# lovesh/bulletproofs-r1cs-gadgets

Measured on AMD Instinct MI355X. Metric: R1CS proofs/sec (Poseidon VSMT-4 depth-32), higher is better.
Workload: dtype int32; 1 GPU; gadget_vsmt_4 sparse-Merkle depth-32 membership (Poseidon 4:1 inverse S-box, 148 rounds); distinct_inputs_steps=9, batch_per_gpu=1024, global_batch=1024, n_multipliers=18656, padded_n=32768, constraints=43330, proof_bytes=1377, proofs_per_device_job=4096, device_jobs=3, jobs_in_flight=2, warmup_steps_run=5, ipa_unfold_rounds=4, table_window_bits=11, table_windows=23, table_format=1, table_bytes=197767468800

## Files before the change

bulletproofs-r1cs-gadgets_amd/csrc/ipa.hpp:

```cpp
#pragma once
#include "msm_run.hpp"
static void* host_stage_alloc(size_t n);
static void host_stage_free(void* p);

struct IpaIO {
    const bpr1cs_gens* g;
    uint32_t B, N, lgN, unfold;
    strobe* tr;
    sc* a;
    sc* bb;
    sc* cG;
    sc* cH;
    const sc* qw;
    const ge* qpt;
    uint8_t* LR;
    sc* uk;
    const uint8_t* hs_tab = nullptr;
    const sc* hs_scal = nullptr;
    uint32_t hs_from = 0;
    dev_stream_t tail_stream{};
    uint32_t tail_rounds = 0;
    struct TailKeep {
        DevBuf<sc> a, bb, linv, cross, cpart;
        DevBuf<ge> GH, vwin, vsum, vout;
        DevBuf<ge_cached> vtab;
        DevBuf<uint32_t> vdig;
    }* tail_keep = nullptr;
    DevArena* own_arena = nullptr;
    sc* sG_pre = nullptr; sc* sH_pre = nullptr;
    IpaGeo geo;
    bool fuse_scalars = true;
    ge_cached* vtab_pre = nullptr; size_t vtab_pre_count = 0;
    dev_event_t* tail_event = nullptr;
};
struct IpaEnd {
    dev_stream_t st;
    sc* a; sc* bb;
};
static IpaEnd enqueue_ipa(const IpaIO& io, dev_stream_t st, MsmStats* stats) {
    const bpr1cs_gens* g = io.g;
    const uint32_t B = io.B, N = io.N, lgN = io.lgN;
    const uint32_t baseG = 2, baseH = 2 + g->cap;
    sc* a = io.a; sc* bb = io.bb; sc* cG = io.cG; sc* cH = io.cH;
    DevBuf<sc> cross((size_t)2 * B);
    const uint32_t r = io.unfold < lgN ? io.unfold : lgN;
    DevBuf<sc> sG, sH, cpart;
    DevBuf<ge> GH, vwin, vsum, vout, partial, partialR;
    DevBuf<ge_cached> vtab;
    DevBuf<uint32_t> vdig;
    DevBuf<sc> linv;
    MsmPlan plan;
    uint32_t M = N >> r;
    ge* GHp = nullptr; ge* vwinp = nullptr; ge* vsump = nullptr; ge* voutp = nullptr;
    ge_cached* vtabp = nullptr; uint32_t* vdigp = nullptr; sc* linvp = nullptr; sc* crossp = cross.p;
    sc* sGp = io.sG_pre; sc* sHp = io.sH_pre;
    const bool geo = io.geo.plo != nullptr;
    if ((r > 0 || (geo && lgN > 0)) && !(sGp && sHp)) { sG.alloc((size_t)N * B); sH.alloc((size_t)N * B); sGp = sG.p; sHp = sH.p; }
    const size_t s_bytes = sGp ? (size_t)N * B * sizeof(sc) : 0;
    const uint32_t facT = 1u << r;
    DevBuf<sc> fac;
    const uint32_t hfJ = N >> 8;
    DevBuf<sc> hf;
    if (geo && lgN > 0) {
        fac.alloc((size_t)6 * facT * B);
        if (hfJ) hf.alloc((size_t)2 * hfJ * B);
    }
    const bool fused = geo && B > MSM_LANE_PATH_MAX_PROOFS && io.fuse_scalars;
    MsmGeo mg;
    auto geo_scalars = [&](uint32_t k, const sc* va, const sc* vb) {
        const uint32_t lgNk = lgN - k;
        launch((uint64_t)2 * (k ? 1u << (k - 1) : 1u) * B, K_ipa_fac{fac.p, k ? io.uk + (size_t)(k - 1) * 2 * B : nullptr, io.geo.upad, B, k, facT}, st);
        const sc* hfp = nullptr;
        if (lgNk >= 8 && hfJ) {
            launch((uint64_t)2 * hfJ * B, K_ipa_hf{fac.p, io.geo.phi + (size_t)io.geo.H * B, hf.p, B, hfJ, lgNk - 8, facT}, st);
            hfp = hf.p;
        }
        if (fused) {
            mg.fac = fac.p; mg.hf = hfp; mg.lo1 = io.geo.plo + (size_t)256 * B; mg.hi1 = io.geo.phi + (size_t)io.geo.H * B;
            mg.T = facT; mg.J = hfJ; mg.Nk = N >> k; mg.lgNk = lgNk; mg.n1 = io.geo.n1;
            return;
        }
        launch((uint64_t)N * B, K_ipa_scalars_geo{va, vb, fac.p, hfp, io.geo, sGp, sHp, B, N >> k, lgNk, facT, hfJ}, st);
    };
    const uint32_t VC = 16;
    const uint32_t VC_TAIL = 4;
    bool vb_reuse = false;
    auto finisher = [&](const ge* part, uint32_t nch, const sc* c, uint8_t* out) {
        K_msm_finish f{g->tab.p, g->tc, part, c, io.qw, out, B, nch, 0};
        if (io.qpt) { f.extra2 = nullptr; f.extra_pt = io.qpt; }
        return f;
    };
    uint32_t tail_from = lgN;
    if (io.tail_rounds && io.tail_keep && io.tail_rounds < lgN) {
        tail_from = std::max(lgN - io.tail_rounds, r + 2);
        if ((tail_from - r) & 1u) tail_from++;
    }
    sc* cpartp = nullptr; size_t cpart_n = 0;
    bool handed_off = false;
    auto emit = [&](uint64_t total, const auto& f, bool wave) {
        if (wave) launch_wave(total, f, st);
        else launch(total, f, st);
    };
    for (uint32_t k = 0; k < lgN; k++) {
        uint32_t Nk = N >> k, mk = Nk >> 1;
        if (k == tail_from && k + 1 < lgN) {
            IpaIO::TailKeep& T = *io.tail_keep;
            {
                ArenaScope own(io.own_arena);
                T.a.alloc((size_t)Nk * B); T.bb.alloc((size_t)Nk * B); T.linv.alloc((size_t)2 * B); T.cross.alloc((size_t)2 * B);
                T.GH.alloc((size_t)2 * Nk * B);
                T.vtab.alloc((size_t)VB_MULT * 4 * mk * B); T.vdig.alloc((size_t)VB_WORDS * 4 * mk * B);
                T.vwin.alloc((size_t)2 * VB_WINDOWS * VC_TAIL * B); T.vsum.alloc((size_t)2 * VB_WINDOWS * B); T.vout.alloc((size_t)2 * B);
            }
            dev_d2d(T.a.p, a, (size_t)Nk * B * sizeof(sc), st);
            dev_d2d(T.bb.p, bb, (size_t)Nk * B * sizeof(sc), st);
            dev_d2d(T.linv.p, linvp, (size_t)2 * B * sizeof(sc), st);
            dev_d2d(T.GH.p, GHp, (size_t)Nk * B * sizeof(ge), st);
            dev_d2d(T.GH.p + (size_t)Nk * B, GHp + (size_t)M * B, (size_t)Nk * B * sizeof(ge), st);
            dev_zero(io.a, (size_t)N * B * sizeof(sc), st);
            dev_zero(io.bb, (size_t)N * B * sizeof(sc), st);
            if (s_bytes) { dev_zero(sGp, s_bytes, st); dev_zero(sHp, s_bytes, st); }
            if (vdig.p) dev_zero(vdig.p, vdig.bytes(), st);
            if (cpart.p) dev_zero(cpart.p, cpart.bytes(), st);
            dev_zero(cross.p, cross.bytes(), st);
            handed_off = true;
            a = T.a.p; bb = T.bb.p; linvp = T.linv.p; crossp = T.cross.p; GHp = T.GH.p; M = Nk;
            vtabp = T.vtab.p; vdigp = T.vdig.p; vwinp = T.vwin.p; vsump = T.vsum.p; voutp = T.vout.p;
            cpartp = nullptr; cpart_n = 0;
            if (io.tail_event) {
                dev_event_create(io.tail_event);
                dev_event_record(*io.tail_event, st);
                dev_stream_wait(io.tail_stream, *io.tail_event);
                st = io.tail_stream;
            }
        }
        uint32_t cchunk, CC = pick_chunks(mk, B, std::min<uint32_t>(1u << 18, sum_chunk_cap(B, 2) * B), cchunk);
        if (cpart_n < (size_t)2 * CC * B) {
            if (k >= tail_from && io.tail_keep) {
                ArenaScope own(io.own_arena);
                io.tail_keep->cpart.alloc((size_t)2 * CC * B);
                cpartp = io.tail_keep->cpart.p;
            } else {
                cpart.alloc((size_t)2 * CC * B);
                cpartp = cpart.p;
            }
            cpart_n = (size_t)2 * CC * B;
        }
        emit((uint64_t)CC * B, K_ipa_cross{a, bb, cpartp, B, mk, cchunk, CC}, false);
        launch_sum_partials((uint64_t)2 * B, K_sum_partials{cpartp, crossp, B, CC}, st);
        uint8_t* Lout = io.LR + ((size_t)k * 2 + 0) * B * 32;
        uint8_t* Rout = io.LR + ((size_t)k * 2 + 1) * B * 32;
        if (k < r) {
            if (geo) {
                geo_scalars(k, a, bb);
            } else {
                K_ipa_scalars ks{a, bb, cG, cH, sGp, sHp, B, Nk};
                if (k > 0) ks.uk_prev = io.uk + (size_t)(k - 1) * 2 * B;
                launch((uint64_t)N * B, ks, st);
            }
            uint32_t half = N / 2;
            MsmSeg gL{sGp, half, mk, Nk, mk, baseG, 0}, hL{sHp, half, mk, Nk, 0, baseH, 0};
            MsmSeg gR{sGp, half, mk, Nk, 0, baseG, 0}, hR{sHp, half, mk, Nk, mk, baseH, 0};
            if (fused) {
                gL.scal = gR.scal = a; hL.scal = hR.scal = bb;
                gL.geo = gR.geo = 1; hL.geo = hR.geo = 2;
            }
            const bool hs = k == 0 && io.hs_tab && io.hs_from < mk;
            if (hs) {
                hL.count = io.hs_from;
                gR.count = io.hs_from;
            }
            MsmPlan planR;
            MsmReq rq[2] = {{gL, hL, &partial, &plan, nullptr}, {gR, hR, &partialR, &planR, nullptr}};
            run_msm_multi(g, rq, 2, B, st, stats, fused ? &mg : nullptr);
            K_msm_finish fL = finisher(partial.p, plan.nchunks, crossp, Lout);
            if (hs) { fL.tab2 = io.hs_tab; fL.extra_b = io.hs_scal; }
            launch_finish_pair(fL, finisher(partialR.p, planR.nchunks, crossp + B, Rout), B, st);
        } else {
            if (k == r) {
                const size_t dead = r >= 1 ? (size_t)(N - M) * B * sizeof(sc) : 0;
                const size_t gh_b = (size_t)2 * M * B * sizeof(ge), vwin_b = ((size_t)2 * VB_WINDOWS * VC * B * sizeof(ge) + 255) & ~(size_t)255,
                             vdig_b = (size_t)VB_WORDS * 4 * (M / 2 ? M / 2 : 1) * B * sizeof(uint32_t);
                if (gh_b <= dead) GHp = (ge*)(io.a + (size_t)M * B);
                else { GH.alloc((size_t)2 * M * B); GHp = GH.p; }
                if (vwin_b + vdig_b <= dead) {
                    uint8_t* base = (uint8_t*)(io.bb + (size_t)M * B);
                    vwinp = (ge*)base;
                    vdigp = (uint32_t*)(base + vwin_b);
                } else {
                    vdig.alloc((size_t)VB_WORDS * 4 * (M / 2 ? M / 2 : 1) * B);
                    vwin.alloc((size_t)2 * VB_WINDOWS * VC * B);
                    vdigp = vdig.p; vwinp = vwin.p;
                }
                const sc* fG = cG; const sc* fH = cH;
                if (geo) {
                    geo_scalars(k, nullptr, nullptr);
                    fG = sGp; fH = sHp;
                }
                const uint32_t f_mont = geo ? 0u : 1u;
                if (B <= MSM_LANE_PATH_MAX_PROOFS) {
                    launch_wave((uint64_t)2 * M * B, K_ipa_fold_from_tables{g->tab.p, g->tc, fG, fH, GHp, B, M, N, baseG, baseH, geo ? 1u : 0u}, st);
                } else {
                    MsmLaunch L{};
                    L.B = B; L.nbk = (B + 63u) / 64u; L.njobs = 2;
                    const MsmSeg none{nullptr, 0, 1, 1, 0, 0, 0};
                    L.job[0] = MsmJob{{MsmSeg{fG, N, N, N, 0, baseG, f_mont}, none}, g->tab.p, g->tc, GHp, N / M, M, 1};
                    L.job[1] = MsmJob{{MsmSeg{fH, N, N, N, 0, baseH, f_mont}, none}, g->tab.p, g->tc, GHp + (size_t)M * B, N / M, M, 1};
                    if (fused) {
                        L.job[0].seg[0].scal = nullptr; L.job[0].seg[0].geo = 1;
                        L.job[1].seg[0].scal = nullptr; L.job[1].seg[0].geo = 2;
                        L.geo = mg;
                    }
                    L.wg_end[0] = M * L.nbk; L.wg_end[1] = 2 * M * L.nbk;
                    launch_msm_kernel(g, L, st, stats, (uint64_t)2 * N * B, (uint64_t)2 * N * B * g->tc.windows);
                }
                const size_t vtab_need = (size_t)VB_MULT * 4 * (M / 2 ? M / 2 : 1) * B;
                if (!(io.vtab_pre && io.vtab_pre_count >= vtab_need)) vtab.alloc(vtab_need);
                vsum.alloc((size_t)2 * VB_WINDOWS * B);
                vout.alloc((size_t)2 * B);
                linv.alloc((size_t)2 * B);
                launch((uint64_t)2 * B, K_set_one{linv.p}, st);
                vtabp = vtab.p ? vtab.p : io.vtab_pre; vsump = vsum.p; voutp = vout.p; linvp = linv.p;
            }
            const uint32_t remap = 1u;
            if (!vb_reuse) {
                const uint32_t vcmax = handed_off ? VC_TAIL : VC;
                const uint32_t vc = 2 * mk < vcmax ? 2 * mk : vcmax;
                emit((uint64_t)4 * mk * B, K_ipa_vb_tab{a, bb, GHp, linvp, vtabp, vdigp, B, mk, M}, false);
                emit((uint64_t)2 * VB_WINDOWS * vc * B, K_ipa_vb_win{vtabp, vdigp, vwinp, B, mk, vc, remap, 0}, true);
                emit((uint64_t)2 * VB_WINDOWS * B, K_ge_reduce{vwinp, vsump, B, 2 * VB_WINDOWS * vc, vc}, false);
            } else {
                const uint32_t vcmax = handed_off ? VC_TAIL : VC;
                const uint32_t m0 = 2 * mk, vc = 2 * m0 < vcmax ? 2 * m0 : vcmax;
                emit((uint64_t)4 * m0 * B, K_ipa_vb_dig2{a, bb, linvp, io.uk + (size_t)(k - 1) * 2 * B, vdigp, B, m0}, false);
                emit((uint64_t)2 * VB_WINDOWS * vc * B, K_ipa_vb_win{vtabp, vdigp, vwinp, B, m0, vc, remap, 1}, true);
                emit((uint64_t)2 * VB_WINDOWS * B, K_ge_reduce{vwinp, vsump, B, 2 * VB_WINDOWS * vc, vc}, false);
            }
            emit((uint64_t)2 * B, K_ipa_vb_horner{vsump, voutp, B, 1}, false);
            launch_finish_pair(finisher(voutp, 1, crossp, Lout), finisher(voutp + (size_t)B, 1, crossp + B, Rout), B, st);
        }
        sc* ukk = io.uk + (size_t)k * 2 * B;
        launch_transcript(B, K_transcript_LR{io.tr, Lout, ukk, B}, st);
        emit((uint64_t)mk * B, K_ipa_fold_ab{a, bb, ukk, B, mk}, false);
        if (k + 1 == r && !geo) launch((uint64_t)N * B, K_ipa_update_c{cG, cH, ukk, B, Nk}, st);
        else if (k < r) {}
        else if (!vb_reuse) {
            vb_reuse = k + 1 < lgN;
        } else {
            if (k + 1 < lgN) emit((uint64_t)2 * mk * B, K_ipa_vb_fold2{GHp, io.uk + (size_t)(k - 1) * 2 * B, ukk, linvp, vtabp, B, 2 * mk, M}, false);
            vb_reuse = false;
        }
    }
    if (!handed_off && s_bytes) {
        dev_zero(sGp, s_bytes, st);
        dev_zero(sHp, s_bytes, st);
    }
    if (handed_off) {
        IpaIO::TailKeep& T = *io.tail_keep;
        if (T.vdig.p) dev_zero(T.vdig.p, T.vdig.bytes(), st);
        if (T.cpart.p) dev_zero(T.cpart.p, T.cpart.bytes(), st);
        if (T.cross.p) dev_zero(T.cross.p, T.cross.bytes(), st);
    } else {
        if (vdig.p) dev_zero(vdig.p, vdig.bytes(), st);
        if (cpart.p) dev_zero(cpart.p, cpart.bytes(), st);
        dev_zero(cross.p, cross.bytes(), st);
    }
    return IpaEnd{st, a, bb};
}
```

bulletproofs-r1cs-gadgets_amd/csrc/kernels.hpp:

```cpp
#pragma once
#include "fe.hpp"
#include "sc.hpp"
#include "ge.hpp"
#include "merlin.hpp"
#include "msm_trace.hpp"

struct TabCfg {
    uint32_t W, windows, entries, row, per_base;
    uint32_t stride;
    HD size_t base_bytes() const { return (size_t)per_base * stride; }
};
HD inline TabCfg tab_cfg(uint32_t W) {
    TabCfg t;
    t.W = W;
    t.windows = (252 + W) / W;
    t.entries = 1u << (W - 1);
    t.row = t.entries + 1;
    t.per_base = t.windows * t.row;
    t.stride = 128;
    return t;
}
HD inline int tab_digit(const sc& s, uint32_t k, int& carry, const TabCfg& tc) {
    uint32_t bit = k * tc.W, wi = bit >> 5, sh = bit & 31;
    uint64_t two = (uint64_t)s.v[wi] | ((wi + 1 < 8) ? ((uint64_t)s.v[wi + 1] << 32) : 0);
// ... 807 lines not shown
};

struct K_ct_gather_T {
    const sc* tco;
    const sc* blind;
    sc* out;
    uint32_t B;
    HD void operator()(uint32_t g) const {
        const uint32_t k = g / B, b = g % B;
        const uint32_t ti[5] = {0, 2, 3, 4, 5};
        out[g] = tco[(size_t)ti[k] * B + b];
        out[(size_t)5 * B + g] = blind[(size_t)(3 + k) * B + b];
    }
};
struct K_ct_finish {
    const ge* partial;
    uint32_t nchunks, count;
    uint8_t* out;
    uint32_t B, m;
    HD void operator()(uint32_t g) const {
        ge acc = partial[g];
        for (uint32_t c = 1; c < nchunks; c++) acc = ge_add_ge(acc, partial[(size_t)c * count + g]);
        ge_compress(acc, out + 32 * (m ? (size_t)(g % B) * m + g / B : (size_t)g));
    }
};

struct K_transcript_T {
    strobe* tr;
    const uint8_t* Tc;
    const sc* tco;
    const sc* blind;
    const sc* wV;
    const sc* vbl_m;
    sc* chal;
    sc* txs;
    uint32_t B, m;
    uint64_t padded_n;
    const sc* t2b_pre = nullptr;
    HD void operator()(uint32_t b) const {
        strobe s = tr[b];
        merlin_append(s, "T_1", 3, Tc + ((size_t)0 * B + b) * 32, 32);
        merlin_append(s, "T_3", 3, Tc + ((size_t)1 * B + b) * 32, 32);
        merlin_append(s, "T_4", 3, Tc + ((size_t)2 * B + b) * 32, 32);
        merlin_append(s, "T_5", 3, Tc + ((size_t)3 * B + b) * 32, 32);
        merlin_append(s, "T_6", 3, Tc + ((size_t)4 * B + b) * 32, 32);
        sc u = merlin_challenge_scalar(s, "u", 1);
        sc x = merlin_challenge_scalar(s, "x", 1);
        sc t2b = sc_zero();
        if (t2b_pre) t2b = t2b_pre[b];
        else for (uint32_t j = 0; j < m; j++) t2b = sc_add(t2b, sc_mul(wV[(size_t)j * B + b], vbl_m[(size_t)j * B + b]));
        sc t[6], tb[6];
        for (int k = 0; k < 6; k++) t[k] = tco[(size_t)k * B + b];
        tb[0] = blind[(size_t)3 * B + b]; tb[1] = t2b;
        for (int k = 2; k < 6; k++) tb[k] = blind[(size_t)(2 + k) * B + b];
        sc tx = t[5], txb = tb[5];
        for (int k = 4; k >= 0; k--) {
            tx = sc_add(t[k], sc_mul(x, tx));
            txb = sc_add(tb[k], sc_mul(x, txb));
        }
        tx = sc_mul(x, tx);
        txb = sc_mul(x, txb);
        sc ib = blind[(size_t)0 * B + b], ob = blind[(size_t)1 * B + b], sb = blind[(size_t)2 * B + b];
        sc eb = sc_mul(x, sc_add(ib, sc_mul(x, sc_add(ob, sc_mul(x, sb)))));
        merlin_append_scalar(s, "t_x", 3, tx);
        merlin_append_scalar(s, "t_x_blinding", 12, txb);
        merlin_append_scalar(s, "e_blinding", 10, eb);
        sc w = merlin_challenge_scalar(s, "w", 1);
        merlin_append(s, "dom-sep", 7, (const uint8_t*)"ipp v1", 6);
        merlin_append_u64(s, "n", 1, padded_n);
        tr[b] = s;
        chal[(size_t)CH_U * B + b] = u;
        chal[(size_t)CH_X * B + b] = x;
        chal[(size_t)CH_W * B + b] = w;
        txs[(size_t)0 * B + b] = tx; txs[(size_t)1 * B + b] = txb; txs[(size_t)2 * B + b] = eb;
    }
};

struct K_lr_eval {
    const sc* W;
    const sc* wvec;
    const sc* plo;
    const sc* phi;
    const sc* chal;
    sc* a;
    sc* bb;
    sc* cG;
    sc* cH;
    uint32_t B, H, n;
    HD void operator()(uint32_t g) const {
        uint32_t i = g / B, b = g % B;
        sc yi = pow_lookup(plo, phi, 0, H, B, i, b), yinv = (i < n || cG) ? pow_lookup(plo, phi, 1, H, B, i, b) : sc_zero();
        sc x = chal[(size_t)CH_X * B + b];
        if (i < n) {
            size_t ib = (size_t)i * B + b, nb = (size_t)n * B;
            sc aL = W[ib], aR = W[nb + ib], aO = W[2 * nb + ib], sL = W[3 * nb + ib], sR = W[4 * nb + ib];
            sc wL = wvec[ib], wR = wvec[nb + ib], wO = wvec[2 * nb + ib];
            sc l1 = sc_add(aL, sc_mul(yinv, wR));
            sc r0 = sc_sub(wO, yi), r1 = sc_add(sc_mul(yi, aR), wL), r3 = sc_mul(yi, sR);
            a[g] = sc_mul(x, sc_add(l1, sc_mul(x, sc_add(aO, sc_mul(x, sL)))));
            bb[g] = sc_add(r0, sc_mul(x, sc_add(r1, sc_mul(x, sc_mul(x, r3)))));
            if (cG) {
                cG[g] = sc_one_mont();
                cH[g] = yinv;
            }
        } else {
            a[g] = sc_zero();
            bb[g] = sc_neg(yi);
            if (cG) {
                sc u = chal[(size_t)CH_U * B + b];
                cG[g] = u;
                cH[g] = sc_mul(yinv, u);
            }
        }
    }
};

struct K_ipa_cross {
    const sc* a;
    const sc* bb;
    sc* part;
    uint32_t B, m, chunk, C;
    HD void operator()(uint32_t g) const {
        uint32_t c = g / B, b = g % B;
        uint32_t lo = c * chunk, hi = lo + chunk < m ? lo + chunk : m;
        sc cl = sc_zero(), cr = sc_zero();
        for (uint32_t j = lo; j < hi; j++) {
            size_t jl = (size_t)j * B + b, jh = (size_t)(j + m) * B + b;
            cl = sc_add(cl, sc_mul(a[jl], bb[jh]));
            cr = sc_add(cr, sc_mul(a[jh], bb[jl]));
        }
        part[(size_t)0 * C * B + g] = cl;
        part[(size_t)1 * C * B + g] = cr;
    }
};
struct K_ipa_scalars {
    const sc* a;
    const sc* bb;
    sc* cG;
    sc* cH;
    sc* sG;
    sc* sH;
    uint32_t B, Nk;
    const sc* uk_prev = nullptr;
    HD void operator()(uint32_t g) const {
        uint32_t i = g / B, b = g % B, m = Nk >> 1;
        uint32_t pos = i & (Nk - 1);
        uint32_t partner = pos >= m ? pos - m : pos + m;
        size_t pb = (size_t)partner * B + b;
        sc cg = cG[g], ch = cH[g];
        if (uk_prev) {
            int hi = (i & (2u * Nk - 1u)) >= Nk;
            sc u = uk_prev[b], ui = uk_prev[(size_t)B + b];
            cg = sc_mul(cg, hi ? u : ui);
            ch = sc_mul(ch, hi ? ui : u);
            cG[g] = cg;
            cH[g] = ch;
        }
        sG[g] = sc_from_mont(sc_mul(a[pb], cg));
        sH[g] = sc_from_mont(sc_mul(bb[pb], ch));
    }
};
struct IpaGeo {
    const sc* plo = nullptr;
    const sc* phi = nullptr;
    const sc* upad = nullptr;
    uint32_t H = 0, n1 = 0;
};
struct K_ipa_fac {
    sc* fac;
    const sc* uk;
    const sc* upad;
    uint32_t B, k, T;
    HD static uint32_t brev(uint32_t x, uint32_t bits) {
        uint32_t r = 0;
        for (uint32_t i = 0; i < bits; i++) r |= ((x >> i) & 1u) << (bits - 1u - i);
        return r;
    }
    HD void operator()(uint32_t g) const {
        const uint32_t half = k ? 1u << (k - 1) : 1u;
        const uint32_t b = g % B, ss = g / B, side = ss / half, s = ss % half;
        sc* f = fac + (size_t)side * T * B + b;
        sc* c0 = fac + (size_t)(2 + 2 * side) * T * B + b;
        sc* c1 = c0 + (size_t)T * B;
        const sc up = upad[b];
        if (k == 0) {
            const sc one = sc_one_mont();
            f[0] = one;
            c0[0] = sc_from_mont(one);
            c1[0] = sc_from_mont(sc_mul(one, up));
            return;
        }
        const sc u = uk[b], ui = uk[(size_t)B + b];
        const sc fhi = side ? ui : u, flo = side ? u : ui;
        const sc x = f[(size_t)s * B];
        const sc lo = sc_mul(x, flo), hi = sc_mul(x, fhi);
        f[(size_t)s * B] = lo;
        f[(size_t)(s + half) * B] = hi;
        const uint32_t t_lo = brev(s, k), t_hi = brev(s + half, k);
        c0[(size_t)t_lo * B] = sc_from_mont(lo);
        c1[(size_t)t_lo * B] = sc_from_mont(sc_mul(lo, up));
        c0[(size_t)t_hi * B] = sc_from_mont(hi);
        c1[(size_t)t_hi * B] = sc_from_mont(sc_mul(hi, up));
    }
};
struct K_ipa_hf {
    const sc* fac;
    const sc* phi_yinv;
    sc* hf;
    uint32_t B, J, shift, T;
    HD void operator()(uint32_t g) const {
        uint32_t b = g % B, ej = g / B, e = ej / J, j = ej % J;
        hf[g] = sc_mul(phi_yinv[(size_t)j * B + b], fac[((size_t)(4 + e) * T + (j >> shift)) * B + b]);
    }
};
struct K_ipa_scalars_geo {
    const sc* a;
    const sc* bb;
    const sc* fac;
    const sc* hf;
    IpaGeo geo;
    sc* sG;
    sc* sH;
    uint32_t B, Nk, lgNk, T, J;
    HD void operator()(uint32_t g) const {
        uint32_t i = g / B, b = g % B, m = Nk >> 1;
        uint32_t pos = i & (Nk - 1), t = i >> lgNk;
        uint32_t partner = pos >= m ? pos - m : pos + m;
        size_t pb = (size_t)partner * B + b;
        const uint32_t e = i >= geo.n1 ? 1u : 0u;
        sc cg = fac[((size_t)(2 + e) * T + t) * B + b];
        sc ch;
        if (hf) ch = sc_mul(geo.plo[((size_t)256 + (i & 255u)) * B + b], hf[((size_t)e * J + (i >> 8)) * B + b]);
        else ch = sc_mul(pow_lookup(geo.plo, geo.phi, 1, geo.H, B, i, b), fac[((size_t)(4 + e) * T + t) * B + b]);
        sG[g] = a ? sc_mul(a[pb], cg) : cg;
        sH[g] = a ? sc_mul(bb[pb], ch) : ch;
    }
};
struct K_transcript_LR {
    strobe* tr;
    const uint8_t* LR;
    sc* uk;
    uint32_t B;
    HD void operator()(uint32_t b) const {
        strobe s = tr[b];
        merlin_append(s, "L", 1, LR + ((size_t)0 * B + b) * 32, 32);
        merlin_append(s, "R", 1, LR + ((size_t)1 * B + b) * 32, 32);
        sc u = merlin_challenge_scalar(s, "u", 1);
        tr[b] = s;
        uk[b] = u;
        uk[(size_t)B + b] = sc_invert_var(u);
    }
};
struct K_ipa_fold_ab {
    sc* a;
    sc* bb;
    const sc* uk;
    uint32_t B, m;
    HD void operator()(uint32_t g) const {
        uint32_t b = g % B;
        size_t hi = g + (size_t)m * B;
        sc u = uk[b], ui = uk[(size_t)B + b];
        a[g] = sc_add(sc_mul(a[g], u), sc_mul(ui, a[hi]));
        bb[g] = sc_add(sc_mul(bb[g], ui), sc_mul(u, bb[hi]));
    }
};
struct K_ipa_update_c {
    sc* cG;
    sc* cH;
    const sc* uk;
    uint32_t B, Nk;
    HD void operator()(uint32_t g) const {
        uint32_t i = g / B, b = g % B, m = Nk >> 1;
        int hi = (i & (Nk - 1)) >= m;
        sc u = uk[b], ui = uk[(size_t)B + b];
        cG[g] = sc_mul(cG[g], hi ? u : ui);
        cH[g] = sc_mul(cH[g], hi ? ui : u);
    }
};
struct K_ipa_fold_from_tables {
    const uint8_t* tab;
    TabCfg tc;
    const sc* cG;
    const sc* cH;
    ge* GH;
    uint32_t B, M, N, baseG, baseH;
    uint32_t canonical = 0;
    HD void operator()(uint32_t g0) const {
        uint32_t g = g0;
        const uint32_t nwg = (uint32_t)(((uint64_t)2 * M * B + 63u) / 64u);
        if ((B & 63u) == 0 && (nwg & 7u) == 0) {
            uint32_t wg = g0 >> 6;
            wg = (wg & 7u) * (nwg >> 3) + (wg >> 3);
            g = (wg << 6) | (g0 & 63u);
        }
        uint32_t b = g % B, sj = g / B, side = sj / M, j = sj % M;
        const sc* c = side ? cH : cG;
        uint32_t base0 = side ? baseH : baseG;
        ge acc = ge_identity();
        for (uint32_t i = j; i < N; i += M)
            acc = table_mul_acc_raw(acc, tab + (size_t)(base0 + i) * tc.base_bytes(), canonical ? c[(size_t)i * B + b] : sc_from_mont(c[(size_t)i * B + b]), tc);
        GH[g] = ge_from_table_class(acc);
    }
};
#define VB_W 5u
#define VB_WINDOWS 51u
#define VB_MULT 16u
#define VB_PER_WORD 6u
#define VB_WORDS 9u
HD inline void vb_recode(const sc& s, uint32_t dig[VB_WORDS]) {
#pragma unroll
    for (uint32_t i = 0; i < VB_WORDS; i++) dig[i] = 0;
    int carry = 0;
#pragma unroll
    for (uint32_t wi = 0; wi < VB_WORDS; wi++) {
        uint32_t o = 0;
#pragma unroll
        for (uint32_t k = 0; k < VB_PER_WORD; k++) {
            const uint32_t i = wi * VB_PER_WORD + k;
            if (i < VB_WINDOWS) {
                const uint32_t bit = i * VB_W, w0 = bit >> 5, sh = bit & 31u;
                uint32_t v = s.v[w0] >> sh;
                if (sh + VB_W > 32u && w0 + 1u < 8u) v |= s.v[w0 + 1u] << (32u - sh);
                int d = (int)(v & (VB_MULT * 2u - 1u)) + carry;
                carry = d >= (int)VB_MULT;
                d -= carry << (VB_W);
                o |= ((uint32_t)d & (VB_MULT * 2u - 1u)) << (VB_W * k);
            }
        }
        dig[wi] = o;
    }
}
HD inline int vb_digit(uint32_t word, uint32_t k) {
    int d = (int)((word >> (VB_W * k)) & (VB_MULT * 2u - 1u));
    return d - ((d & (int)VB_MULT) << 1);
}
template <int N>
HD inline ge ge_dbln(const ge& p) {
    ge q = p;
#pragma unroll
    for (int i = 0; i + 1 < N; i++) q = ge_p1p1_to_p2(ge_dbl_c(q));
    return ge_p1p1_to_p3(ge_dbl_c(q));
}
struct K_ipa_vb_tab {
    const sc* a;
    const sc* bb;
    const ge* GH;
    const sc* linv;
    ge_cached* vtab;
    uint32_t* vdig;
    uint32_t B, m, M;
    HD void operator()(uint32_t g) const {
        uint32_t b = g % B, wj = g / B, w = wj / m, j = wj % m;
        uint32_t side = w & 1u;
        const sc* sv = side ? bb : a;
        const ge* pv = side ? GH + (size_t)M * B : GH;
        uint32_t s_hi = (w == 1u) | (w == 2u), p_hi = (w == 0u) | (w == 3u);
        sc s = sc_from_mont(sc_mul(sv[(size_t)(j + s_hi * m) * B + b], linv[(size_t)side * B + b]));
        ge P = pv[(size_t)(j + p_hi * m) * B + b];
        size_t stride = (size_t)4 * m * B;
        ge_cached c1 = ge_to_cached(P);
        ge_cached* T = vtab + g;
        T[0] = c1;
        ge q = P;
        for (uint32_t e = 1; e < VB_MULT; e++) {
            q = ge_add(q, c1);
            T[(size_t)e * stride] = ge_to_cached(q);
        }
        uint32_t dig[VB_WORDS];
        vb_recode(s, dig);
#pragma unroll
        for (uint32_t i = 0; i < VB_WORDS; i++) vdig[(size_t)i * stride + g] = dig[i];
    }
};
HD inline uint32_t vb_win_index(uint32_t g0, uint32_t B, uint32_t VC, uint32_t remap, uint32_t& out, uint32_t& win, uint32_t& c, uint32_t& b) {
    b = g0 % B;
    uint32_t r0 = g0 / B;
    c = r0 % VC;
    uint32_t ow = r0 / VC;
    win = ow % VB_WINDOWS;
    out = ow / VB_WINDOWS;
    const uint32_t nbk = B >> 6, nwg = 2u * VB_WINDOWS * VC * nbk;
    if (remap && (B & 63u) == 0 && (nwg & 7u) == 0) {
        uint32_t wg = g0 >> 6;
        wg = (wg & 7u) * (nwg >> 3) + (wg >> 3);
        win = wg % VB_WINDOWS;
        uint32_t r1 = wg / VB_WINDOWS, bk = r1 % nbk;
        r1 /= nbk;
        c = r1 % VC;
        out = r1 / VC;
        b = (bk << 6) | (g0 & 63u);
    }
    return ((out * VB_WINDOWS + win) * VC + c) * B + b;
}
struct K_ipa_vb_win {
    const ge_cached* vtab;
    const uint32_t* vdig;
    ge* part;
    uint32_t B, m, VC, remap;
    uint32_t skip;
    HD void operator()(uint32_t g0) const {
        uint32_t out, win, c, b;
        const uint32_t g = vb_win_index(g0, B, VC, remap, out, win, c, b);
        uint32_t total = 2 * m, per = (total + VC - 1) / VC;
        uint32_t lo = c * per, hi = lo + per < total ? lo + per : total;
        size_t stride = (size_t)4 * m * B;
        const uint32_t dw = win / VB_PER_WORD, dk = win - dw * VB_PER_WORD;
        ge acc = ge_identity();
        for (uint32_t o = lo; o < hi; o++) {
            size_t t;
            if (!skip) t = ((size_t)(2 * out) * m + o) * B + b;
            else {
                const uint32_t h = m >> 1, q = o / h, jj = o - q * h;
                const uint32_t w = q == 0 ? 2u : q == 1 ? 0u : q == 2 ? 1u : 3u;
                const uint32_t up = (q < 2) ? (out == 0) : (out != 0);
                t = ((size_t)w * m + jj + up * h) * B + b;
            }
            int d = vb_digit(vdig[(size_t)dw * stride + t], dk);
            if (d != 0) {
                int mag = d < 0 ? -d : d;
                ge_cached e = vtab[(size_t)(mag - 1) * stride + t];
                acc = ge_addsub(acc, e, d < 0);
            }
        }
        part[g] = acc;
    }
};
struct K_ipa_vb_horner {
    const ge* part;
    ge* out;
    uint32_t B, VC;
    HD void operator()(uint32_t g) const {
        uint32_t b = g % B, o = g / B;
        ge acc = ge_identity();
        for (int w = (int)VB_WINDOWS - 1; w >= 0; w--) {
            if (w != (int)VB_WINDOWS - 1) acc = ge_dbln<(int)VB_W>(acc);
            const ge* p = part + (((size_t)o * VB_WINDOWS + (uint32_t)w) * VC) * B + b;
            for (uint32_t c = 0; c < VC; c++) acc = ge_add_ge(acc, p[(size_t)c * B]);
        }
        out[g] = acc;
    }
};
struct K_ipa_vb_dig2 {
    const sc* a;
    const sc* bb;
    const sc* linv;
    const sc* uk;
    uint32_t* vdig;
    uint32_t B, m;
    HD void operator()(uint32_t g) const {
        uint32_t b = g % B, wj = g / B, w = wj / m, j = wj % m, h = m >> 1;
        uint32_t side = w & 1u, hi = (w == 0u) | (w == 3u);
        const sc* sv = side ? bb : a;
        uint32_t idx = j >= h ? j - h : j + h;
        sc fac = sc_mul(linv[(size_t)side * B + b], uk[(size_t)((side ^ hi) ? 0u : 1u) * B + b]);
        sc s = sc_from_mont(sc_mul(sv[(size_t)idx * B + b], fac));
        uint32_t dig[VB_WORDS];
        vb_recode(s, dig);
        const size_t stride = (size_t)4 * m * B;
#pragma unroll
        for (uint32_t i = 0; i < VB_WORDS; i++) vdig[(size_t)i * stride + g] = dig[i];
    }
};
HD inline ge vb_add_digit(const ge& acc, uint32_t word, uint32_t k, const ge_cached* T, size_t stride) {
    int d = vb_digit(word, k);
    if (d == 0) return acc;
    int mag = d < 0 ? -d : d;
    ge_cached e = T[(size_t)(mag - 1) * stride];
    return ge_addsub(acc, e, d < 0);
}
struct K_ipa_vb_fold2 {
    ge* GH;
    const sc* uk0;
    const sc* uk1;
    sc* linv;
    const ge_cached* vtab;
    uint32_t B, m, M;
    HD void operator()(uint32_t g) const {
        const uint32_t h = m >> 1;
        uint32_t b = g % B, sj = g / B, side = sj / h, j = sj % h;
        ge* P = GH + (size_t)side * M * B;
        const uint32_t fi = side ? 1u : 0u;
        sc f0 = uk0[(size_t)fi * B + b], f1 = uk1[(size_t)fi * B + b];
        sc w0m = sc_mul(f0, f0), w1m = sc_mul(f1, f1);
        uint32_t p0[VB_WORDS], p1[VB_WORDS], p01[VB_WORDS];
        vb_recode(sc_from_mont(w0m), p0);
        vb_recode(sc_from_mont(w1m), p1);
        vb_recode(sc_from_mont(sc_mul(w0m, w1m)), p01);
        const size_t stride = (size_t)4 * m * B;
        const uint32_t w_lo = side ? 1u : 2u, w_hi = side ? 3u : 0u;
        const ge_cached* T0 = vtab + ((size_t)w_hi * m + j) * B + b;
        const ge_cached* T1 = vtab + ((size_t)w_lo * m + j + h) * B + b;
        const ge_cached* T01 = vtab + ((size_t)w_hi * m + j + h) * B + b;
        ge acc = ge_identity();
#pragma unroll
        for (int wi = (int)VB_WORDS - 1; wi >= 0; wi--) {
            const uint32_t d0 = p0[wi], d1 = p1[wi], d01 = p01[wi];
            for (int k = (int)VB_PER_WORD - 1; k >= 0; k--) {
                const uint32_t i = (uint32_t)wi * VB_PER_WORD + (uint32_t)k;
                if (i >= VB_WINDOWS) continue;
                if (i + 1u < VB_WINDOWS) acc = ge_dbln<(int)VB_W>(acc);
                acc = vb_add_digit(acc, d0, (uint32_t)k, T0, stride);
                acc = vb_add_digit(acc, d1, (uint32_t)k, T1, stride);
                acc = vb_add_digit(acc, d01, (uint32_t)k, T01, stride);
            }
        }
        ge lo = P[(size_t)j * B + b];
        P[(size_t)j * B + b] = ge_add_ge(lo, acc);
        if (j == 0) {
            const uint32_t gi = side ? 0u : 1u;
            linv[(size_t)side * B + b] = sc_mul(linv[(size_t)side * B + b], sc_mul(uk0[(size_t)gi * B + b], uk1[(size_t)gi * B + b]));
        }
    }
};
struct K_set_one {
    sc* p;
    HD void operator()(uint32_t g) const { p[g] = sc_one_mont(); }
};
#define VCH_Y 0
#define VCH_Z 1
#define VCH_YINV 2
#define VCH_U 3
#define VCH_X 4
#define VCH_W 5
#define VCH_R 6
#define VCH_A 7
#define VCH_B 8
#define VCH_TX 9
#define VCH_TXB 10
#define VCH_EB 11
#define VCH_COUNT 12

HD inline int bytes_are_zero32(const uint8_t* p) {
    uint8_t o = 0;
    for (int i = 0; i < 32; i++) o |= p[i];
    return o == 0;
}
HD inline int scalar_bytes_canonical(const uint8_t* p) {
    sc a = sc_load_raw(p);
    for (int i = 7; i >= 0; i--) {
        if (a.v[i] < SC_L[i]) return 1;
        if (a.v[i] > SC_L[i]) return 0;
    }
    return 0;
}
struct K_verify_transcript {
    const uint8_t* label;
    uint32_t label_len;
    const uint8_t* proofs;
    const uint8_t* Vc;
    const uint8_t* seeds;
    sc* chal;
    sc* uk;
    int* fail;
    uint32_t B, m, lgN, plen;
    uint64_t padded_n;
    uint8_t* bind = nullptr;
    HD void operator()(uint32_t b) const {
        const uint8_t* pf = proofs + (size_t)b * plen;
        int bad = pf[0] != 0;
        const uint8_t* el = pf + 1;
        bad |= !scalar_bytes_canonical(el + 8 * 32) | !scalar_bytes_canonical(el + 9 * 32) | !scalar_bytes_canonical(el + 10 * 32);
        bad |= !scalar_bytes_canonical(el + (11 + 2 * lgN) * 32) | !scalar_bytes_canonical(el + (12 + 2 * lgN) * 32);
        strobe s;
        merlin_new(s, label, label_len);
        merlin_append(s, "dom-sep", 7, (const uint8_t*)"r1cs v1", 7);
        for (uint32_t j = 0; j < m; j++) merlin_append(s, "V", 1, Vc + ((size_t)b * m + j) * 32, 32);
        merlin_append_u64(s, "m", 1, m);
        bad |= bytes_are_zero32(el) | bytes_are_zero32(el + 32) | bytes_are_zero32(el + 64);
        merlin_append(s, "A_I1", 4, el, 32);
        merlin_append(s, "A_O1", 4, el + 32, 32);
        merlin_append(s, "S1", 2, el + 64, 32);
        merlin_append(s, "dom-sep", 7, (const uint8_t*)"r1cs-1phase", 11);
        uint8_t id[32];
        for (int i = 0; i < 32; i++) id[i] = 0;
        merlin_append(s, "A_I2", 4, id, 32);
        merlin_append(s, "A_O2", 4, id, 32);
        merlin_append(s, "S2", 2, id, 32);
        sc y = merlin_challenge_scalar(s, "y", 1);
        sc z = merlin_challenge_scalar(s, "z", 1);
        for (int k = 0; k < 5; k++) bad |= bytes_are_zero32(el + (3 + k) * 32);
        merlin_append(s, "T_1", 3, el + 3 * 32, 32);
        merlin_append(s, "T_3", 3, el + 4 * 32, 32);
        merlin_append(s, "T_4", 3, el + 5 * 32, 32);
        merlin_append(s, "T_5", 3, el + 6 * 32, 32);
        merlin_append(s, "T_6", 3, el + 7 * 32, 32);
        sc u = merlin_challenge_scalar(s, "u", 1);
        sc x = merlin_challenge_scalar(s, "x", 1);
        merlin_append(s, "t_x", 3, el + 8 * 32, 32);
        merlin_append(s, "t_x_blinding", 12, el + 9 * 32, 32);
        merlin_append(s, "e_blinding", 10, el + 10 * 32, 32);
        sc w = merlin_challenge_scalar(s, "w", 1);
        merlin_append(s, "dom-sep", 7, (const uint8_t*)"ipp v1", 6);
        merlin_append_u64(s, "n", 1, padded_n);
        for (uint32_t k = 0; k < lgN; k++) {
            const uint8_t* Lp = el + (11 + 2 * k) * 32;
            bad |= bytes_are_zero32(Lp) | bytes_are_zero32(Lp + 32);
            merlin_append(s, "L", 1, Lp, 32);
            merlin_append(s, "R", 1, Lp + 32, 32);
            sc uu = merlin_challenge_scalar(s, "u", 1);
            uk[((size_t)k * 2 + 0) * B + b] = uu;
        }
        sc yinv;
        {
            sc acc = y;
            for (uint32_t k = 0; k < lgN; k++) {
                uk[((size_t)k * 2 + 1) * B + b] = acc;
                acc = sc_mul(acc, uk[((size_t)k * 2 + 0) * B + b]);
            }
            sc inv = sc_invert_var(acc);
            for (uint32_t k = lgN; k-- > 0;) {
                const sc before = uk[((size_t)k * 2 + 1) * B + b];
                uk[((size_t)k * 2 + 1) * B + b] = sc_mul(inv, before);
                inv = sc_mul(inv, uk[((size_t)k * 2 + 0) * B + b]);
            }
            yinv = inv;
        }
        if (bind) {
            strobe t = s;
            merlin_append(t, "ipp_a", 5, el + (11 + 2 * lgN) * 32, 32);
            merlin_append(t, "ipp_b", 5, el + (12 + 2 * lgN) * 32, 32);
            merlin_challenge_bytes(t, "bpr1cs-bind", 11, bind + 32 * (size_t)b, 32);
        }
        merlin_rng_finalize(s, seeds + 32 * (size_t)b);
        sc r = merlin_rng_scalar(s);
        sc* c = chal;
        c[(size_t)VCH_Y * B + b] = y; c[(size_t)VCH_Z * B + b] = z; c[(size_t)VCH_YINV * B + b] = yinv;
        c[(size_t)VCH_U * B + b] = u; c[(size_t)VCH_X * B + b] = x; c[(size_t)VCH_W * B + b] = w; c[(size_t)VCH_R * B + b] = r;
        c[(size_t)VCH_TX * B + b] = sc_mont_from_bytes_mod_order(el + 8 * 32);
        c[(size_t)VCH_TXB * B + b] = sc_mont_from_bytes_mod_order(el + 9 * 32);
        c[(size_t)VCH_EB * B + b] = sc_mont_from_bytes_mod_order(el + 10 * 32);
        c[(size_t)VCH_A * B + b] = sc_mont_from_bytes_mod_order(el + (11 + 2 * lgN) * 32);
        c[(size_t)VCH_B * B + b] = sc_mont_from_bytes_mod_order(el + (12 + 2 * lgN) * 32);
        fail[b] = bad;
    }
};
struct K_verify_gh {
    const sc* wvec;
    const sc* plo;
    const sc* phi;
    const sc* chal;
    const sc* uk;
    sc* gs;
    sc* hs;
    sc* dpart;
    uint32_t B, H, n, N, lgN;
    HD void operator()(uint32_t g) const {
        uint32_t i = g / B, b = g % B;
        sc s = sc_one_mont(), sinv = sc_one_mont();
        for (uint32_t k = 0; k < lgN; k++) {
            uint32_t bit = (i >> (lgN - 1 - k)) & 1u;
            sc uu = uk[((size_t)k * 2 + 0) * B + b], ui = uk[((size_t)k * 2 + 1) * B + b];
            s = sc_mul(s, bit ? uu : ui);
            sinv = sc_mul(sinv, bit ? ui : uu);
        }
        sc yinv = pow_lookup(plo, phi, 1, H, B, i, b);
        sc x = chal[(size_t)VCH_X * B + b], a = chal[(size_t)VCH_A * B + b], bb = chal[(size_t)VCH_B * B + b];
        sc u_or_1 = i < n ? sc_one_mont() : chal[(size_t)VCH_U * B + b];
        sc wL = sc_zero(), wR = sc_zero(), wO = sc_zero();
        if (i < n) {
            size_t ib = (size_t)i * B + b, nb = (size_t)n * B;
            wL = wvec[ib]; wR = wvec[nb + ib]; wO = wvec[2 * nb + ib];
        }
        sc ynwR = sc_mul(yinv, wR);
        sc gi = sc_mul(u_or_1, sc_sub(sc_mul(x, ynwR), sc_mul(a, s)));
        sc hi = sc_mul(u_or_1, sc_sub(sc_mul(yinv, sc_sub(sc_add(sc_mul(x, wL), wO), sc_mul(bb, sinv))), sc_one_mont()));
        gs[g] = sc_from_mont(gi);
        hs[g] = sc_from_mont(hi);
        dpart[g] = sc_mul(ynwR, wL);
    }
};
struct K_verify_bscalars {
    const sc* chal;
    const sc* wc;
    const sc* delta;
    sc* out;
    uint32_t B;
    HD void operator()(uint32_t b) const {
        const sc* c = chal;
        sc x = c[(size_t)VCH_X * B + b], w = c[(size_t)VCH_W * B + b], r = c[(size_t)VCH_R * B + b];
        sc a = c[(size_t)VCH_A * B + b], bb = c[(size_t)VCH_B * B + b], tx = c[(size_t)VCH_TX * B + b];
        sc xx = sc_mul(x, x);
        sc cB = sc_add(sc_mul(w, sc_sub(tx, sc_mul(a, bb))), sc_mul(r, sc_sub(sc_mul(xx, sc_add(wc[b], delta[b])), tx)));
        sc cBb = sc_sub(sc_neg(c[(size_t)VCH_EB * B + b]), sc_mul(r, c[(size_t)VCH_TXB * B + b]));
        out[b] = cB;
        out[(size_t)B + b] = cBb;
    }
};
struct K_verify_points {
    const uint8_t* proofs;
    const uint8_t* Vc;
    const sc* chal;
    const sc* uk;
    const sc* wV;
    ge* out;
    int* fail;
    uint32_t B, m, lgN, plen;
    const sc* rho = nullptr;
    ge_cached* vtab = nullptr;
    uint32_t* vdig = nullptr;
    HD void operator()(uint32_t g) const {
        uint32_t p = g / B, b = g % B;
        const uint8_t* el = proofs + (size_t)b * plen + 1;
        const sc* c = chal;
        sc x = c[(size_t)VCH_X * B + b], r = c[(size_t)VCH_R * B + b];
        sc xx = sc_mul(x, x), xxx = sc_mul(xx, x), rxx = sc_mul(r, xx);
        const uint8_t* pt;
        sc s;
        if (p < 3) { pt = el + 32 * p; s = p == 0 ? x : (p == 1 ? xx : xxx); }
        else if (p < 3 + m) { uint32_t j = p - 3; pt = Vc + ((size_t)b * m + j) * 32; s = sc_mul(wV[(size_t)j * B + b], rxx); }
        else if (p < 8 + m) {
            uint32_t k = p - 3 - m;
            pt = el + 32 * (3 + k);
            sc t = sc_mul(r, x);
            if (k >= 1) t = sc_mul(rxx, x);
            if (k >= 2) t = sc_mul(rxx, xx);
            if (k >= 3) t = sc_mul(rxx, xxx);
            if (k >= 4) t = sc_mul(sc_mul(rxx, xx), xx);
            s = t;
        } else {
            uint32_t q = p - 8 - m, k = q >> 1, isR = q & 1u;
            pt = el + 32 * (11 + 2 * k + isR);
            sc uu = uk[((size_t)k * 2 + isR) * B + b];
            s = sc_mul(uu, uu);
        }
        ge P;
        const bool bad = !ge_decompress(pt, P);
        if (bad) { fail[b] = 1; P = ge_identity(); }
        if (rho) s = sc_mul(s, rho[b]);
        if (vtab) {
            const size_t T = (size_t)(8 + m + 2 * lgN) * B;
            ge_cached c1 = ge_to_cached(P);
            vtab[g] = c1;
            ge q = P;
            for (uint32_t e = 1; e < VB_MULT; e++) {
                q = ge_add(q, c1);
                vtab[(size_t)e * T + g] = ge_to_cached(q);
            }
            uint32_t dig[VB_WORDS];
            vb_recode(bad ? sc_zero() : sc_from_mont(s), dig);
#pragma unroll
            for (uint32_t i = 0; i < VB_WORDS; i++) vdig[(size_t)i * T + g] = dig[i];
            return;
        }
        out[g] = bad ? ge_identity() : ge_scalarmul_naf(P, sc_from_mont(s));
    }
};
#define BATCH_LEAF 32u
struct K_batch_leaf {
    const uint8_t* bind;
    uint8_t* leaf;
    uint32_t B;
    HD void operator()(uint32_t g) const {
        strobe t;
        const char lab[] = "bpr1cs batch leaf";
        merlin_new(t, (const uint8_t*)lab, sizeof(lab) - 1);
        merlin_append_u64(t, "leaf", 4, g);
        uint32_t lo = g * BATCH_LEAF, hi = lo + BATCH_LEAF < B ? lo + BATCH_LEAF : B;
        for (uint32_t b = lo; b < hi; b++) merlin_append(t, "proof", 5, bind + 32 * (size_t)b, 32);
        merlin_challenge_bytes(t, "leaf", 4, leaf + 32 * (size_t)g, 32);
    }
};
struct K_batch_digest {
    const uint8_t* seed;
    const uint8_t* leaf;
    uint8_t* digest;
    uint64_t index_base;
    uint32_t B;
    HD void operator()(uint32_t) const {
        strobe t;
        const char lab[] = "bpr1cs batch verify";
        merlin_new(t, (const uint8_t*)lab, sizeof(lab) - 1);
        merlin_append(t, "seed", 4, seed, 32);
        merlin_append_u64(t, "base", 4, index_base);
        merlin_append_u64(t, "count", 5, B);
        const uint32_t leaves = (B + BATCH_LEAF - 1) / BATCH_LEAF;
        for (uint32_t g = 0; g < leaves; g++) merlin_append(t, "leaf", 4, leaf + 32 * (size_t)g, 32);
        merlin_challenge_bytes(t, "digest", 6, digest, 32);
    }
};
struct K_batch_weights {
    const uint8_t* digest;
    sc* rho;
    uint64_t index_base;
    HD void operator()(uint32_t b) const {
        strobe t;
        const char lab[] = "bpr1cs batch weight";
// ... 275 lines not shown
```

Baseline: 2977 proofs/s.

## Fold IPA generators with shared per-block scalars and unit first block

```diff
diff --git a/bulletproofs-r1cs-gadgets_amd/csrc/ipa.hpp b/bulletproofs-r1cs-gadgets_amd/csrc/ipa.hpp
--- a/bulletproofs-r1cs-gadgets_amd/csrc/ipa.hpp
+++ b/bulletproofs-r1cs-gadgets_amd/csrc/ipa.hpp
@@ -22,6 +22,7 @@
     uint32_t tail_rounds = 0;
     struct TailKeep {
         DevBuf<sc> a, bb, linv, cross, cpart;
+        DevBuf<sc> ypow;
         DevBuf<ge> GH, vwin, vsum, vout;
         DevBuf<ge_cached> vtab;
         DevBuf<uint32_t> vdig;
@@ -67,9 +68,12 @@
     }
     const bool fused = geo && B > MSM_LANE_PATH_MAX_PROOFS && io.fuse_scalars;
     MsmGeo mg;
+    auto geo_fac = [&](uint32_t k) {
+        launch((uint64_t)2 * (k ? 1u << (k - 1) : 1u) * B, K_ipa_fac{fac.p, k ? io.uk + (size_t)(k - 1) * 2 * B : nullptr, io.geo.upad, B, k, facT}, st);
+    };
     auto geo_scalars = [&](uint32_t k, const sc* va, const sc* vb) {
         const uint32_t lgNk = lgN - k;
-        launch((uint64_t)2 * (k ? 1u << (k - 1) : 1u) * B, K_ipa_fac{fac.p, k ? io.uk + (size_t)(k - 1) * 2 * B : nullptr, io.geo.upad, B, k, facT}, st);
+        geo_fac(k);
         const sc* hfp = nullptr;
         if (lgNk >= 8 && hfJ) {
             launch((uint64_t)2 * hfJ * B, K_ipa_hf{fac.p, io.geo.phi + (size_t)io.geo.H * B, hf.p, B, hfJ, lgNk - 8, facT}, st);
@@ -85,6 +89,10 @@
     const uint32_t VC = 16;
     const uint32_t VC_TAIL = 4;
     bool vb_reuse = false;
+    const bool unit = geo && r >= 1 && r < lgN && B > MSM_LANE_PATH_MAX_PROOFS && io.geo.n1 >= M;
+    YPos ypos;
+    DevBuf<sc> fsc;
+    DevBuf<uint32_t> fidx;
     auto finisher = [&](const ge* part, uint32_t nch, const sc* c, uint8_t* out) {
         K_msm_finish f{g->tab.p, g->tc, part, c, io.qw, out, B, nch, 0};
         if (io.qpt) { f.extra2 = nullptr; f.extra_pt = io.qpt; }
@@ -111,6 +119,12 @@
                 T.GH.alloc((size_t)2 * Nk * B);
                 T.vtab.alloc((size_t)VB_MULT * 4 * mk * B); T.vdig.alloc((size_t)VB_WORDS * 4 * mk * B);
                 T.vwin.alloc((size_t)2 * VB_WINDOWS * VC_TAIL * B); T.vsum.alloc((size_t)2 * VB_WINDOWS * B); T.vout.alloc((size_t)2 * B);
+                if (ypos.lo) T.ypow.alloc((size_t)(256 + std::max<uint32_t>(Nk >> 8, 1u)) * B);
+            }
+            if (ypos.lo) {
+                dev_d2d(T.ypow.p, ypos.lo, (size_t)256 * B * sizeof(sc), st);
+                dev_d2d(T.ypow.p + (size_t)256 * B, ypos.hi, (size_t)std::max<uint32_t>(Nk >> 8, 1u) * B * sizeof(sc), st);
+                ypos.lo = T.ypow.p; ypos.hi = T.ypow.p + (size_t)256 * B;
             }
             dev_d2d(T.a.p, a, (size_t)Nk * B * sizeof(sc), st);
             dev_d2d(T.bb.p, bb, (size_t)Nk * B * sizeof(sc), st);
@@ -193,7 +207,15 @@
                     vdigp = vdig.p; vwinp = vwin.p;
                 }
                 const sc* fG = cG; const sc* fH = cH;
-                if (geo) {
+                if (unit) {
+                    geo_fac(k);
+                    fsc.alloc((size_t)4 * facT * B);
+                    fidx.alloc((size_t)N - M);
+                    linv.alloc((size_t)2 * B);
+                    launch((uint64_t)2 * facT * B, K_ipa_fold_scal{fac.p, io.uk, io.geo.plo + (size_t)256 * B, io.geo.phi + (size_t)io.geo.H * B, fsc.p, linv.p, B, facT, r, M}, st);
+                    launch((uint64_t)N - M, K_ipa_fold_idx{fidx.p, M, io.geo.n1}, st);
+                    ypos.lo = io.geo.plo + (size_t)256 * B; ypos.hi = io.geo.phi + (size_t)io.geo.H * B;
+                } else if (geo) {
                     geo_scalars(k, nullptr, nullptr);
                     fG = sGp; fH = sHp;
                 }
@@ -206,33 +228,41 @@
                     const MsmSeg none{nullptr, 0, 1, 1, 0, 0, 0};
                     L.job[0] = MsmJob{{MsmSeg{fG, N, N, N, 0, baseG, f_mont}, none}, g->tab.p, g->tc, GHp, N / M, M, 1};
                     L.job[1] = MsmJob{{MsmSeg{fH, N, N, N, 0, baseH, f_mont}, none}, g->tab.p, g->tc, GHp + (size_t)M * B, N / M, M, 1};
-                    if (fused) {
+                    uint32_t per_side = N;
+                    if (unit) {
+                        per_side = N - M;
+                        L.job[0].seg[0] = MsmSeg{fsc.p, per_side, 1, 1, 0, baseG + M, MSM_CANONICAL, fidx.p, 1};
+                        L.job[1].seg[0] = MsmSeg{fsc.p + (size_t)2 * facT * B, per_side, 1, 1, 0, baseH + M, MSM_CANONICAL, fidx.p, 1};
+                    } else if (fused) {
                         L.job[0].seg[0].scal = nullptr; L.job[0].seg[0].geo = 1;
                         L.job[1].seg[0].scal = nullptr; L.job[1].seg[0].geo = 2;
                         L.geo = mg;
                     }
                     L.wg_end[0] = M * L.nbk; L.wg_end[1] = 2 * M * L.nbk;
-                    launch_msm_kernel(g, L, st, stats, (uint64_t)2 * N * B, (uint64_t)2 * N * B * g->tc.windows);
+                    launch_msm_kernel(g, L, st, stats, (uint64_t)2 * per_side * B, (uint64_t)2 * per_side * B * g->tc.windows);
+                    if (unit) launch((uint64_t)2 * M * B, K_ipa_fold_unit{g->tab.p, g->tc, GHp, B, M, baseG, baseH}, st);
                 }
                 const size_t vtab_need = (size_t)VB_MULT * 4 * (M / 2 ? M / 2 : 1) * B;
                 if (!(io.vtab_pre && io.vtab_pre_count >= vtab_need)) vtab.alloc(vtab_need);
                 vsum.alloc((size_t)2 * VB_WINDOWS * B);
                 vout.alloc((size_t)2 * B);
-                linv.alloc((size_t)2 * B);
-                launch((uint64_t)2 * B, K_set_one{linv.p}, st);
+                if (!unit) {
+                    linv.alloc((size_t)2 * B);
+                    launch((uint64_t)2 * B, K_set_one{linv.p}, st);
+                }
                 vtabp = vtab.p ? vtab.p : io.vtab_pre; vsump = vsum.p; voutp = vout.p; linvp = linv.p;
             }
             const uint32_t remap = 1u;
             if (!vb_reuse) {
                 const uint32_t vcmax = handed_off ? VC_TAIL : VC;
                 const uint32_t vc = 2 * mk < vcmax ? 2 * mk : vcmax;
-                emit((uint64_t)4 * mk * B, K_ipa_vb_tab{a, bb, GHp, linvp, vtabp, vdigp, B, mk, M}, false);
+                emit((uint64_t)4 * mk * B, K_ipa_vb_tab{a, bb, GHp, linvp, vtabp, vdigp, B, mk, M, ypos}, false);
                 emit((uint64_t)2 * VB_WINDOWS * vc * B, K_ipa_vb_win{vtabp, vdigp, vwinp, B, mk, vc, remap, 0}, true);
                 emit((uint64_t)2 * VB_WINDOWS * B, K_ge_reduce{vwinp, vsump, B, 2 * VB_WINDOWS * vc, vc}, false);
             } else {
                 const uint32_t vcmax = handed_off ? VC_TAIL : VC;
                 const uint32_t m0 = 2 * mk, vc = 2 * m0 < vcmax ? 2 * m0 : vcmax;
-                emit((uint64_t)4 * m0 * B, K_ipa_vb_dig2{a, bb, linvp, io.uk + (size_t)(k - 1) * 2 * B, vdigp, B, m0}, false);
+                emit((uint64_t)4 * m0 * B, K_ipa_vb_dig2{a, bb, linvp, io.uk + (size_t)(k - 1) * 2 * B, vdigp, B, m0, ypos}, false);
                 emit((uint64_t)2 * VB_WINDOWS * vc * B, K_ipa_vb_win{vtabp, vdigp, vwinp, B, m0, vc, remap, 1}, true);
                 emit((uint64_t)2 * VB_WINDOWS * B, K_ge_reduce{vwinp, vsump, B, 2 * VB_WINDOWS * vc, vc}, false);
             }
@@ -247,7 +277,7 @@
         else if (!vb_reuse) {
             vb_reuse = k + 1 < lgN;
         } else {
-            if (k + 1 < lgN) emit((uint64_t)2 * mk * B, K_ipa_vb_fold2{GHp, io.uk + (size_t)(k - 1) * 2 * B, ukk, linvp, vtabp, B, 2 * mk, M}, false);
+            if (k + 1 < lgN) emit((uint64_t)2 * mk * B, K_ipa_vb_fold2{GHp, io.uk + (size_t)(k - 1) * 2 * B, ukk, linvp, vtabp, B, 2 * mk, M, ypos}, false);
             vb_reuse = false;
         }
     }
diff --git a/bulletproofs-r1cs-gadgets_amd/csrc/kernels.hpp b/bulletproofs-r1cs-gadgets_amd/csrc/kernels.hpp
--- a/bulletproofs-r1cs-gadgets_amd/csrc/kernels.hpp
+++ b/bulletproofs-r1cs-gadgets_amd/csrc/kernels.hpp
@@ -1133,6 +1133,51 @@
         GH[g] = ge_from_table_class(acc);
     }
 };
+struct K_ipa_fold_scal {
+    const sc* fac;
+    const sc* uk;
+    const sc* lo1;
+    const sc* hi1;
+    sc* out;
+    sc* linv;
+    uint32_t B, T, r, M;
+    HD void operator()(uint32_t g) const {
+        const uint32_t b = g % B, st = g / B, side = st / T, t = st % T;
+        sc inv0 = sc_one_mont();
+        for (uint32_t k = 0; k < r; k++) inv0 = sc_mul(inv0, uk[((size_t)k * 2 + side) * B + b]);
+        if (side) {
+            const uint32_t p = t * M;
+            inv0 = sc_mul(inv0, sc_mul(lo1[(size_t)(p & 255u) * B + b], hi1[(size_t)(p >> 8) * B + b]));
+        }
+        for (uint32_t e = 0; e < 2; e++)
+            out[(((size_t)side * T + t) * 2 + e) * B + b] = sc_mul(inv0, fac[((size_t)(2 + 2 * side + e) * T + t) * B + b]);
+        if (t == 0) linv[(size_t)side * B + b] = fac[(size_t)side * T * B + b];
+    }
+};
+struct K_ipa_fold_idx {
+    uint32_t* sidx;
+    uint32_t M, n1;
+    HD void operator()(uint32_t o) const {
+        const uint32_t i = o + M;
+        sidx[o] = 2u * (i / M) + (i >= n1 ? 1u : 0u);
+    }
+};
+struct K_ipa_fold_unit {
+    const uint8_t* tab;
+    TabCfg tc;
+    ge* GH;
+    uint32_t B, M, baseG, baseH;
+    HD void operator()(uint32_t g) const {
+        const uint32_t sj = g / B, side = sj / M, j = sj % M;
+        const uint8_t* row = tab + (size_t)((side ? baseH : baseG) + j) * tc.base_bytes();
+        GH[g] = ge_from_table_class(ge_madd_t(GH[g], ge_niels_load(row + tc.stride), 0));
+    }
+};
+struct YPos {
+    const sc* lo = nullptr;
+    const sc* hi = nullptr;
+    HD sc at(uint32_t p, uint32_t B, uint32_t b) const { return sc_mul(lo[(size_t)(p & 255u) * B + b], hi[(size_t)(p >> 8) * B + b]); }
+};
 #define VB_W 5u
 #define VB_WINDOWS 51u
 #define VB_MULT 16u
@@ -1180,13 +1225,16 @@
     ge_cached* vtab;
     uint32_t* vdig;
     uint32_t B, m, M;
+    YPos ypos;
     HD void operator()(uint32_t g) const {
         uint32_t b = g % B, wj = g / B, w = wj / m, j = wj % m;
         uint32_t side = w & 1u;
         const sc* sv = side ? bb : a;
         const ge* pv = side ? GH + (size_t)M * B : GH;
         uint32_t s_hi = (w == 1u) | (w == 2u), p_hi = (w == 0u) | (w == 3u);
-        sc s = sc_from_mont(sc_mul(sv[(size_t)(j + s_hi * m) * B + b], linv[(size_t)side * B + b]));
+        sc sm = sc_mul(sv[(size_t)(j + s_hi * m) * B + b], linv[(size_t)side * B + b]);
+        if (side && ypos.lo) sm = sc_mul(sm, ypos.at(j + p_hi * m, B, b));
+        sc s = sc_from_mont(sm);
         ge P = pv[(size_t)(j + p_hi * m) * B + b];
         size_t stride = (size_t)4 * m * B;
         ge_cached c1 = ge_to_cached(P);
@@ -1278,12 +1326,14 @@
     const sc* uk;
     uint32_t* vdig;
     uint32_t B, m;
+    YPos ypos;
     HD void operator()(uint32_t g) const {
         uint32_t b = g % B, wj = g / B, w = wj / m, j = wj % m, h = m >> 1;
         uint32_t side = w & 1u, hi = (w == 0u) | (w == 3u);
         const sc* sv = side ? bb : a;
         uint32_t idx = j >= h ? j - h : j + h;
         sc fac = sc_mul(linv[(size_t)side * B + b], uk[(size_t)((side ^ hi) ? 0u : 1u) * B + b]);
+        if (side && ypos.lo) fac = sc_mul(fac, ypos.at(j + hi * m, B, b));
         sc s = sc_from_mont(sc_mul(sv[(size_t)idx * B + b], fac));
         uint32_t dig[VB_WORDS];
         vb_recode(s, dig);
@@ -1306,6 +1356,7 @@
     sc* linv;
     const ge_cached* vtab;
     uint32_t B, m, M;
+    YPos ypos;
     HD void operator()(uint32_t g) const {
         const uint32_t h = m >> 1;
         uint32_t b = g % B, sj = g / B, side = sj / h, j = sj % h;
@@ -1313,6 +1364,7 @@
         const uint32_t fi = side ? 1u : 0u;
         sc f0 = uk0[(size_t)fi * B + b], f1 = uk1[(size_t)fi * B + b];
         sc w0m = sc_mul(f0, f0), w1m = sc_mul(f1, f1);
+        if (side && ypos.lo) { w0m = sc_mul(w0m, ypos.at(m, B, b)); w1m = sc_mul(w1m, ypos.at(h, B, b)); }
         uint32_t p0[VB_WORDS], p1[VB_WORDS], p01[VB_WORDS];
         vb_recode(sc_from_mont(w0m), p0);
         vb_recode(sc_from_mont(w1m), p1);
```

Result: faster. 3010 proofs/s, median of 6 (+1.1%).
